# g1mv/density

Hardware: NVIDIA H100
Metric: chameleon_encode_input_GBps (higher is better)
Workload: dtype u32

## Files before the change

### density_b200/csrc/chameleon_encode.cu

```cuda
#include <cstdio>
#include "common.cuh"
#include "encode_internal.cuh"

namespace dns {
namespace cham {

constexpr int TILE_Q = 4096;
__device__ __forceinline__ bool bit_test(const uint32_t* bm, uint32_t i) { return (bm[i >> 5] >> (i & 31)) & 1u; }

constexpr int F6_THREADS = 512, F6_QPT = 8;
constexpr int F6_NW = F6_THREADS / 32, F6_WQ = 32 * F6_QPT;
static_assert(F6_THREADS * F6_QPT == TILE_Q, "tile geometry");
constexpr int F6_MB_SLOTS = 4096, F6_MB_CAP = 4;
constexpr int F6_SEC_SLOTS = 64, F6_SEC_CAP = 16;
#ifdef DNS_PHASE_TIMING
__device__ long long g_f6_ph[8];
#define F6_PH(k) { if (threadIdx.x == 0 && blockIdx.x == 77) { long long tn = clock64(); g_f6_ph[k] += tn - f6_tprev; f6_tprev = tn; } }
#define F6_PH_DECL long long f6_tprev = clock64();
#else
#define F6_PH(k)
#define F6_PH_DECL
#endif
constexpr uint32_t F6_TOUCHED = 1u << 12, F6_DROPPED = 1u << 13;
struct Flag6Smem {
// ... 247 lines not shown
                }
                if (hit) atomicOr(&S.sigw[buf][pos >> 5], 1u << (pos & 31));
            }
            f6_append_unres(unres, run_q0 + pos, r.x, &S.unres_count, unres_run);
        }
    }
    __syncthreads();
    F6_PH(3)
}

__global__ void __launch_bounds__(F6_THREADS, 1)
cham_flag_pass6(const uint32_t* __restrict__ in, uint64_t nquads, uint32_t tiles_total, uint32_t nruns,
                uint32_t* __restrict__ sigw_g, uint2* __restrict__ unres, uint32_t* __restrict__ unres_count,
                uint32_t* __restrict__ final_tab, const uint8_t* __restrict__ copymap, const Status* __restrict__ gate)
{
    if (gate && !(gate->nonquiet && !gate->converged)) return;
    extern __shared__ __align__(16) unsigned char smem_raw[];
    Flag6Smem& S = *reinterpret_cast<Flag6Smem*>(smem_raw);
    const uint32_t tid = threadIdx.x, lane = tid & 31, warp = tid >> 5;
    const uint32_t run = blockIdx.x;
    const uint64_t t_begin = (uint64_t)run * tiles_total / nruns;
    const uint64_t t_end = (uint64_t)(run + 1) * tiles_total / nruns;
    uint2* __restrict__ unres_run = unres + (size_t)run * 65536;
    const uint32_t pos0 = warp * F6_WQ + lane;
    const uint32_t ntile_run = (uint32_t)(t_end - t_begin);
    const uint64_t q_begin = t_begin * TILE_Q;
    const uint64_t q_end64 = (t_end * TILE_Q < nquads) ? t_end * TILE_Q : nquads;
    const uint32_t run_quads = q_begin < q_end64 ? (uint32_t)(q_end64 - q_begin) : 0u;
    const uint32_t* __restrict__ rin = in + q_begin;
    uint32_t* __restrict__ rsig = sigw_g + t_begin * (TILE_Q / 32);
// ... 56 lines not shown
    for (uint32_t i = tid; i < 65536; i += F6_THREADS) {
        const uint32_t v = S.tab[i];
        const uint32_t tch = (v != 0 || bit_test(S.vbit, i)) ? 0x10000u : 0u;
        final_tab[(size_t)run * 65536 + i] = v | tch;
    }
    if (tid == 0) unres_count[run] = S.unres_count < 65536u ? S.unres_count : 65536u;
#ifdef DNS_PHASE_TIMING
    if (tid == 0 && run == 77 && ntile_run) { const long long nt = ntile_run;
        printf("f6 run %u tiles %lld cycles/tile: A %lld B %lld C+deposit %lld D+S4 %lld  overflow tiles %lld dirty/tile %lld\n", run, nt, g_f6_ph[0] / nt, g_f6_ph[1] / nt,
               g_f6_ph[2] / nt, g_f6_ph[3] / nt, g_f6_ph[6], g_f6_ph[7] / nt);
        for (int k = 0; k < 8; ++k) g_f6_ph[k] = 0; }
#endif
}

__device__ __forceinline__ bool gate_open(const Status* g) { return !g || (g->nonquiet && !g->converged); }

__global__ void cham_carry_scan(const uint32_t* __restrict__ final_tab, const uint32_t* __restrict__ init, int init_untouched,
                                uint32_t nruns, uint32_t* __restrict__ carry, uint32_t* __restrict__ table_out,
                                const Status* __restrict__ gate = nullptr) {
    if (!gate_open(gate)) return;
    uint32_t hb = blockIdx.x * blockDim.x + threadIdx.x;
    if (hb >= 65536) return;
    uint32_t c = init ? init[hb] : ((hb == 0 && !init_untouched) ? 0x10000u : 0u);
    for (uint32_t r = 0; r < nruns; ++r) {
        if (carry) carry[(size_t)r * 65536 + hb] = c;
        uint32_t v = final_tab[(size_t)r * 65536 + hb];
        if (v & 0x10000u) c = v;
    }
    if (table_out) table_out[hb] = c;
}

__global__ void cham_resolve(const uint2* __restrict__ unres, const uint32_t* __restrict__ unres_count,
                             const uint32_t* __restrict__ carry, uint32_t tiles_total, uint32_t nruns,
                             uint32_t* __restrict__ sigw_g, const Status* __restrict__ gate = nullptr) {
    if (!gate_open(gate)) return;
    const uint32_t run = blockIdx.y;
    const uint32_t n = unres_count[run];
    const uint64_t run_q0 = ((uint64_t)run * tiles_total / nruns) * TILE_Q;
    for (uint32_t i = blockIdx.x * blockDim.x + threadIdx.x; i < n; i += gridDim.x * blockDim.x) {
        uint2 e = unres[(size_t)run * 65536 + i];
        uint32_t c = carry[(size_t)run * 65536 + (e.y & 0xFFFFu)];
        if ((c & 0x10000u) && (c & 0xFFFFu) == (e.y >> 16)) {
            uint64_t gq = run_q0 + e.x;
            atomicOr(&sigw_g[gq >> 5], 1u << (gq & 31));
        }
    }
}

struct ProtSmem {
    uint16_t tab[65536];
    uint32_t vbit[2048];
};

__global__ void __launch_bounds__(1024, 1)
cham_protected_pass(const uint32_t* __restrict__ in, uint64_t nbytes, const Status* __restrict__ status, int only_if_nonquiet,
                    uint32_t* __restrict__ sigw_g, uint8_t* __restrict__ copymap) {
    if (only_if_nonquiet && !(status->nonquiet && !status->converged)) return;
    extern __shared__ __align__(16) unsigned char smem_raw[];
    ProtSmem& S = *reinterpret_cast<ProtSmem*>(smem_raw);
    const uint32_t tid = threadIdx.x, lane = tid & 31;
    {
        uint4 z = make_uint4(0, 0, 0, 0);
        uint4* t4 = reinterpret_cast<uint4*>(S.tab);
        for (uint32_t i = tid; i < 65536 * 2 / 16; i += blockDim.x) t4[i] = z;
        for (uint32_t i = tid; i < 2048; i += blockDim.x) S.vbit[i] = (i == 0) ? 1u : 0u;
    }
    __syncthreads();
    if (tid >= 32) return;

    const uint64_t nquads = nbytes / 4;
    const uint64_t nblocks = (nbytes + 255) / 256;
// ... 80 lines not shown
        atomicAdd(counter, 1u);
        const unsigned int target = (epoch + 1) * nctas;
        while (atomicAdd(counter, 0u) < target) { __nanosleep(64); }
        __threadfence();
    }
    ++epoch;
    __syncthreads();
}

__device__ unsigned long long g_prot_dbg[16][2];

__global__ void __launch_bounds__(PI_THREADS)
prot_iterate(const uint32_t* __restrict__ sigw_g, uint64_t nbytes, uint64_t nblocks, uint32_t nseg, Status* __restrict__ st, int it,
             uint8_t* __restrict__ inc, uint8_t* __restrict__ cm_old, uint8_t* __restrict__ cm_new,
             uint32_t* __restrict__ in_state, uint32_t* __restrict__ out_state, uint16_t* __restrict__ ptab) {
    if (!gate_open(st)) return;
    __shared__ uint32_t s_state[1024], s_in[1024];
    __shared__ uint8_t s_inc[PSEG], s_cm[PSEG];
    __shared__ uint32_t s_cur, s_redo;
    const uint32_t tid = threadIdx.x;
    const uint64_t gtid = (uint64_t)blockIdx.x * PI_THREADS + tid, gsz = (uint64_t)gridDim.x * PI_THREADS;
    unsigned int epoch = 0;
    unsigned int* bar = &st->barrier[it & 7];

    if (sigw_g)
        for (uint64_t b = gtid; b < nblocks; b += gsz)
            if (!(it && cm_old[b])) inc[b] = (nbytes - b * 256 >= 256) && (__popc(sigw_g[2 * b]) + __popc(sigw_g[2 * b + 1]) <= 4);
    if (gtid == 0) { st->relax_changed[0] = 0; st->relax_changed[1] = 0; st->iter_changed = 0; st->pad2[0] = 0; }
    if (gtid < 16 && it == 0) { g_prot_dbg[gtid][0] = ~0ull; g_prot_dbg[gtid][1] = 0; }
    grid_barrier(bar, gridDim.x, epoch);
// ... 144 lines not shown
    }
    grid_barrier(bar, gridDim.x, epoch);
    const bool converged = *((volatile unsigned int*)&st->iter_changed) == 0;
    if (!converged || it == 0)
        for (uint64_t b = gtid; b < nblocks; b += gsz) cm_old[b] = __ldcg(&cm_new[b]);
    grid_barrier(bar, gridDim.x, epoch);
    if (gtid == 0 && converged) st->converged = 1;
}

__device__ __forceinline__ uint32_t block_out_bytes(uint64_t b, uint64_t nbytes, uint32_t hits, bool copied) {
    const uint64_t boff = b * 256;
    const uint32_t blen = (uint32_t)((nbytes - boff < 256) ? (nbytes - boff) : 256);
    return copied ? blen : 8 + blen - 2 * hits;
}

__global__ void cham_tile_sizes(const uint32_t* __restrict__ sigw_g, const uint8_t* __restrict__ copymap, uint64_t nbytes,
                                uint64_t nblocks, uint32_t ntiles, int use_copymap_if_nonquiet, int check_quiet, int assume_prev_inc,
                                Status* __restrict__ status, uint32_t* __restrict__ tile_bytes) {
    const uint32_t lane = threadIdx.x & 31;
    const uint32_t tile = blockIdx.x * (blockDim.x >> 5) + (threadIdx.x >> 5);
    if (tile >= ntiles) return;
    if (use_copymap_if_nonquiet && !check_quiet && !status->nonquiet) return;
    const bool use_cm = copymap && (!use_copymap_if_nonquiet || status->nonquiet);
    uint32_t sum = 0, incm[2];
#pragma unroll
    for (int k = 0; k < 2; ++k) {
        const uint64_t b = (uint64_t)tile * 64 + k * 32 + lane;
        uint32_t sz = 0; bool inc = false;
        if (b < nblocks) {
            const bool copied = use_cm && copymap[b];
            const uint32_t hits = __popc(sigw_g[2 * b]) + __popc(sigw_g[2 * b + 1]);
            sz = block_out_bytes(b, nbytes, hits, copied);
            inc = !copied && sz >= 256 && (nbytes - b * 256 >= 256);
        }
        sum += sz;
        incm[k] = __ballot_sync(0xFFFFFFFFu, inc);
    }
#pragma unroll
    for (int d = 16; d; d >>= 1) sum += __shfl_xor_sync(0xFFFFFFFFu, sum, d);
    if (lane == 0) tile_bytes[tile] = sum;
    if (check_quiet && lane == 0) {
        bool prev = assume_prev_inc != 0;
        if (tile > 0) {
            const uint64_t b = (uint64_t)tile * 64 - 1;
            const uint32_t hits = __popc(sigw_g[2 * b]) + __popc(sigw_g[2 * b + 1]);
            prev = (8 + 256 - 2 * hits) >= 256;
        }
        const uint64_t m = ((uint64_t)incm[1] << 32) | incm[0];
        const uint64_t pairs = m & ((m << 1) | (prev ? 1ull : 0ull));
        if (pairs) {
            atomicOr(&status->nonquiet, 1u);
            atomicMin(&status->first_nonquiet_block, (unsigned long long)tile * 64 + (__ffsll((long long)pairs) - 1));
        }
    }
}

constexpr int SCAN_T = 1024;
constexpr int SCAN_PER = 4;
constexpr int SCAN_G = SCAN_T * SCAN_PER;

__device__ __forceinline__ uint64_t block_exclusive_scan_u64(uint64_t v, uint64_t* s_warp, uint64_t* total) {
    const uint32_t lane = threadIdx.x & 31, warp = threadIdx.x >> 5;
    uint64_t incl = v;
#pragma unroll
    for (int d = 1; d < 32; d <<= 1) { uint64_t u = __shfl_up_sync(0xFFFFFFFFu, incl, d); if (lane >= (uint32_t)d) incl += u; }
    if (lane == 31) s_warp[warp] = incl;
    __syncthreads();
    if (warp == 0) {
        uint64_t w = (lane < (blockDim.x >> 5)) ? s_warp[lane] : 0;
        uint64_t wi = w;
#pragma unroll
        for (int d = 1; d < 32; d <<= 1) { uint64_t u = __shfl_up_sync(0xFFFFFFFFu, wi, d); if (lane >= (uint32_t)d) wi += u; }
        s_warp[lane] = wi - w;
        if (lane == 31) s_warp[32] = wi;
    }
    __syncthreads();
    if (total) *total = s_warp[32];
    return incl - v + s_warp[warp];
}

__global__ void __launch_bounds__(SCAN_T) scan_groups_local(const uint32_t* __restrict__ tile_bytes, uint32_t ntiles,
                                                           uint32_t* __restrict__ tile_local, uint64_t* __restrict__ group_total) {
    __shared__ uint64_t s_warp[33];
    const uint32_t base = blockIdx.x * SCAN_G + threadIdx.x * SCAN_PER;
    uint32_t v[SCAN_PER]; uint64_t sum = 0;
#pragma unroll
    for (int k = 0; k < SCAN_PER; ++k) { v[k] = (base + k < ntiles) ? tile_bytes[base + k] : 0u; sum += v[k]; }
    uint64_t tot;
    uint64_t ex = block_exclusive_scan_u64(sum, s_warp, &tot);
#pragma unroll
    for (int k = 0; k < SCAN_PER; ++k) { if (base + k < ntiles) tile_local[base + k] = (uint32_t)ex; ex += v[k]; }
    if (threadIdx.x == 0) group_total[blockIdx.x] = tot;
}

__global__ void __launch_bounds__(SCAN_T) scan_group_totals(const uint64_t* __restrict__ group_total, uint32_t ngroups,
                                                           uint64_t* __restrict__ group_off, Status* __restrict__ status,
                                                           uint64_t cap, uint64_t* __restrict__ d_out_size) {
    __shared__ uint64_t s_warp[33];
    __shared__ uint64_t s_carry;
    if (threadIdx.x == 0) s_carry = 0;
    __syncthreads();
    for (uint32_t base = 0; base < ngroups; base += SCAN_T) {
        uint32_t i = base + threadIdx.x;
        uint64_t v = (i < ngroups) ? group_total[i] : 0;
        uint64_t tot;
        uint64_t ex = block_exclusive_scan_u64(v, s_warp, &tot);
        if (i < ngroups) group_off[i] = s_carry + ex;
        __syncthreads();
        if (threadIdx.x == 0) s_carry += tot;
        __syncthreads();
    }
    if (threadIdx.x == 0) {
// ... 48 lines not shown
        if (FULL || (uint32_t)j < nv) {
            const bool hit = (fl >> j) & 1u;
            const uint32_t hsh = prod_hash(hash_prod(qs[j]));
            st_u16(p, hit ? hsh : (qs[j] & 0xFFFFu));
            if (!hit) st_u16(p + 2, qs[j] >> 16);
            p += hit ? 2 : 4;
        }
    }
}

template <bool AL16>
__global__ void __launch_bounds__(EM_THREADS)
cham_emit(const uint32_t* __restrict__ in, uint64_t nbytes, uint64_t nblocks, const uint32_t* __restrict__ sigw_g,
          const uint8_t* __restrict__ copymap, int use_copymap_if_nonquiet, const Status* __restrict__ status,
          const uint32_t* __restrict__ tile_local, const uint64_t* __restrict__ group_off, uint8_t* __restrict__ out) {
    if (status->error) return;
    __shared__ __align__(16) uint8_t s_stage[EM_STAGE];
    __shared__ uint32_t s_off[65];
    __shared__ uint32_t s_sig[128];
    __shared__ uint8_t s_copied[64];
    __shared__ uint32_t s_wsum[2];
    const uint32_t tid = threadIdx.x, lane = tid & 31, warp = tid >> 5;
    const uint32_t tile = blockIdx.x;
    const bool use_cm = copymap && (!use_copymap_if_nonquiet || status->nonquiet);
    const uint64_t tile_off = group_off[tile / SCAN_G] + tile_local[tile];
    const uint64_t nquads = nbytes / 4;
    const uint64_t tq0 = (uint64_t)tile * 4096;
    const bool full = tq0 + 4096 <= nquads;
    const uint32_t nvalid_tile = full ? 4096u : (uint32_t)(nquads > tq0 ? nquads - tq0 : 0);
    uint4 qv[4];
// ... 314 lines not shown
    L->unres = take((size_t)nruns_max * 65536 * sizeof(uint2));
    L->unres_count = take((size_t)nruns_max * sizeof(uint32_t));
    L->final_tab = take((size_t)nruns_max * 65536 * sizeof(uint32_t));
    L->carry = take((size_t)nruns_max * 65536 * sizeof(uint32_t));
    L->total = off;
    return off;
}

static cudaError_t set_smem_attrs_once() {
    static bool done = false;
    static cudaError_t err = cudaSuccess;
    if (!done) {
        err = cudaFuncSetAttribute(cham_flag_pass6, cudaFuncAttributeMaxDynamicSharedMemorySize, (int)sizeof(Flag6Smem));
        if (err == cudaSuccess)
            err = cudaFuncSetAttribute(cham_protected_pass, cudaFuncAttributeMaxDynamicSharedMemorySize, (int)sizeof(ProtSmem));
        done = true;
    }
    return err;
}

static cudaError_t prot_iterate_coop(int ctas, cudaStream_t stream, const uint32_t* sigw, uint64_t nbytes, uint64_t nblocks, uint32_t nseg, Status* st, int it,
                                     uint8_t* inc, uint8_t* cm_old, uint8_t* cm_new, uint32_t* in_state, uint32_t* out_state, uint16_t* ptab) {
    void* args[] = {&sigw, &nbytes, &nblocks, &nseg, &st, &it, &inc, &cm_old, &cm_new, &in_state, &out_state, &ptab};
    return cudaLaunchCooperativeKernel(reinterpret_cast<const void*>(prot_iterate), dim3((unsigned)ctas), dim3(PI_THREADS), args, 0, stream);
}

cudaError_t prot_debug_read(unsigned long long* out32) { return cudaMemcpyFromSymbol(out32, g_prot_dbg, sizeof(unsigned long long) * 32); }

size_t prot_state_bytes(uint64_t nseg_max) { return (2 * (nseg_max + 2) + 64) * sizeof(uint32_t) + prot_table_elems(nseg_max) * sizeof(uint16_t); }

uint32_t cham_pick_runs(size_t nbytes, int num_sms) {
    const uint64_t nblocks = (nbytes + 255) / 256;
    const uint64_t ntiles = (nblocks + 63) / 64;
    uint64_t r = ntiles / 16;
    if (r < 1) r = 1;
    if (r > (uint64_t)num_sms) r = num_sms;
    return (uint32_t)r;
}

// ... 8 lines not shown
        ntiles = (uint32_t)((nblocks + 63) / 64); ngroups = (ntiles + SCAN_G - 1) / SCAN_G;
        nseg = (uint32_t)((nblocks + PSEG - 1) / PSEG); ngrp = (nseg + PC_GROUP - 1) / PC_GROUP;
        st = at<Status>(ws, L.status); sigw = at<uint32_t>(ws, L.sigw);
        copymap = ws + L.copymap; copymap2 = ws + L.copymap2; incb = ws + L.incb;
        seg_state = at<uint32_t>(ws, L.seg_state);
        tile_bytes = at<uint32_t>(ws, L.tile_bytes); tile_local = at<uint32_t>(ws, L.tile_local);
        group_total = at<uint64_t>(ws, L.group_total); group_off = at<uint64_t>(ws, L.group_off);
        unres = at<uint2>(ws, L.unres); unres_count = at<uint32_t>(ws, L.unres_count);
        final_tab = at<uint32_t>(ws, L.final_tab); carry = at<uint32_t>(ws, L.carry);
        in_state = seg_state; out_state = seg_state + (nseg + 1);
        ptab = reinterpret_cast<uint16_t*>(seg_state + 2 * (nseg + 1));
        gin = reinterpret_cast<uint32_t*>(ptab); T = ptab + 2 * (ngrp + 2); GT = T + (size_t)nseg * PC_NC;
    }
};

static void launch_flag_pass(const ChamBufs& B, const uint8_t* d_in, uint32_t nruns, const uint8_t* copymap, const Status* gate, cudaStream_t stream,
                             uint64_t* launches) {
    cham_flag_pass6<<<nruns, F6_THREADS, sizeof(Flag6Smem), stream>>>(reinterpret_cast<const uint32_t*>(d_in), B.nquads, B.ntiles, nruns, B.sigw, B.unres,
                                                                      B.unres_count, B.final_tab, copymap, gate);
    ++*launches;
}
static void launch_carry_resolve(const ChamBufs& B, uint32_t nruns, const uint32_t* d_carry_in, const Status* gate, cudaStream_t stream,
                                 uint64_t* launches) {
    cham_carry_scan<<<65536 / 256, 256, 0, stream>>>(B.final_tab, d_carry_in, 0, nruns, B.carry, nullptr, gate);
    cham_resolve<<<dim3(32, nruns), 256, 0, stream>>>(B.unres, B.unres_count, B.carry, B.ntiles, nruns, B.sigw, gate);
    *launches += 2;
}
static void launch_export_fold(const ChamBufs& B, uint32_t nruns, uint32_t* d_table_out, const Status* gate, cudaStream_t stream, uint64_t* launches) {
    cham_carry_scan<<<65536 / 256, 256, 0, stream>>>(B.final_tab, nullptr, 1, nruns, nullptr, d_table_out, gate);
    ++*launches;
}
static cudaError_t sizes_scan_emit(const ChamBufs& B, const uint8_t* d_in, const uint8_t* copymap, int use_copymap_if_nonquiet, bool al16_ok,
                                   uint8_t* d_out, size_t cap, uint64_t* d_out_size, cudaStream_t stream, uint64_t* launches, cudaEvent_t* ev) {
    if (copymap) {
        cham_tile_sizes<<<(B.ntiles + 7) / 8, 256, 0, stream>>>(B.sigw, copymap, B.nbytes, B.nblocks, B.ntiles, use_copymap_if_nonquiet, 0, 0, B.st, B.tile_bytes);
        ++*launches;
    }
    cudaError_t e = scan_tiles_launch(B.tile_bytes, B.ntiles, B.tile_local, B.group_total, B.group_off, B.ngroups, B.st, (uint64_t)cap, d_out_size, stream);
    if (e != cudaSuccess) return e;
    *launches += 2;
    if (ev) cudaEventRecord(ev[2], stream);
    const uint32_t* in32 = reinterpret_cast<const uint32_t*>(d_in);
    if (al16_ok && (reinterpret_cast<uintptr_t>(d_in) & 15u) == 0)
        cham_emit<true><<<B.ntiles, EM_THREADS, 0, stream>>>(in32, B.nbytes, B.nblocks, B.sigw, copymap, use_copymap_if_nonquiet, B.st, B.tile_local, B.group_off, d_out);
    else
        cham_emit<false><<<B.ntiles, EM_THREADS, 0, stream>>>(in32, B.nbytes, B.nblocks, B.sigw, copymap, use_copymap_if_nonquiet, B.st, B.tile_local, B.group_off, d_out);
    ++*launches;
    if (ev) cudaEventRecord(ev[3], stream);
    return cudaGetLastError();
}

cudaError_t cham_encode_phase1(const uint8_t* d_in, size_t nbytes, uint8_t* ws, const ChamLayout& L, uint32_t nruns,
                               uint32_t* d_table_out, cudaStream_t stream, uint64_t* launches, cudaEvent_t* ev) {
    cudaError_t e = set_smem_attrs_once();
    if (e != cudaSuccess) return e;
    const ChamBufs B(ws, L, nbytes);
    e = cudaMemsetAsync(B.st, 0, sizeof(Status), stream);
    if (e == cudaSuccess) e = cudaMemsetAsync(&B.st->first_nonquiet_block, 0xFF, sizeof(unsigned long long), stream);
    if (e != cudaSuccess) return e;
    if (B.nblocks == 0) return cudaSuccess;
    if (ev) cudaEventRecord(ev[0], stream);
    launch_flag_pass(B, d_in, nruns, nullptr, nullptr, stream, launches);
    if (ev) cudaEventRecord(ev[1], stream);
    if (d_table_out) launch_export_fold(B, nruns, d_table_out, nullptr, stream, launches);
    return cudaGetLastError();
}

static cudaError_t cham_phase2_begin(const ChamBufs& B, uint32_t nruns, const uint32_t* d_carry_in, bool assume_prev_inc, cudaStream_t stream,
                                     uint64_t* launches) {
    launch_carry_resolve(B, nruns, d_carry_in, nullptr, stream, launches);
    cham_tile_sizes<<<(B.ntiles + 7) / 8, 256, 0, stream>>>(B.sigw, nullptr, B.nbytes, B.nblocks, B.ntiles, 0, 1, assume_prev_inc ? 1 : 0, B.st, B.tile_bytes);
    ++*launches;
    return cudaGetLastError();
}

static cudaError_t cham_phase2_rounds(const ChamBufs& B, const uint8_t* d_in, uint32_t nruns, const uint32_t* d_carry_in, int it_first, int it_last,
                                      bool reset_barriers, int num_sms, cudaStream_t stream, uint64_t* launches) {
    const int num_ctas = num_sms > 0 ? num_sms : 1;
    if (it_last - it_first >= 8) return cudaErrorInvalidValue;
    if (reset_barriers) {
        cudaError_t e = cudaMemsetAsync(B.st->barrier, 0, sizeof(B.st->barrier), stream);
        if (e != cudaSuccess) return e;
    }
    for (int it = it_first; it <= it_last; ++it) {
        if (it > 0) {
            launch_flag_pass(B, d_in, nruns, B.copymap, B.st, stream, launches);
            launch_carry_resolve(B, nruns, d_carry_in, B.st, stream, launches);
        }
        cudaError_t le = prot_iterate_coop(num_ctas, stream, B.sigw, B.nbytes, B.nblocks, B.nseg, B.st, it, B.incb, B.copymap, B.copymap2, B.in_state,
                                           B.out_state, B.ptab);
        if (le != cudaSuccess) return le;
        ++*launches;
    }
    return cudaGetLastError();
}

static cudaError_t cham_phase2_finish(const ChamBufs& B, const uint8_t* d_in, uint8_t* d_out, size_t cap, uint64_t* d_out_size, bool with_copy_map,
                                      bool inorder_fallback, cudaStream_t stream, uint64_t* launches, cudaEvent_t* ev) {
    if (with_copy_map && inorder_fallback) {
        cham_protected_pass<<<1, 1024, sizeof(ProtSmem), stream>>>(reinterpret_cast<const uint32_t*>(d_in), B.nbytes, B.st, 1, B.sigw, B.copymap);
        ++*launches;
    }
    return sizes_scan_emit(B, d_in, with_copy_map ? B.copymap : nullptr, 1, true, d_out, cap, d_out_size, stream, launches, ev);
}

static cudaError_t cham_phase2_needs_more(const ChamBufs& B, cudaStream_t stream, bool* more) {
    Status h;
    cudaError_t e = cudaMemcpyAsync(&h, B.st, sizeof h, cudaMemcpyDeviceToHost, stream);
    if (e == cudaSuccess) e = cudaStreamSynchronize(stream);
    if (e != cudaSuccess) return e;
    *more = h.nonquiet && !h.converged && !h.error;
    return cudaSuccess;
}

constexpr int PROT_ITERS = 4;

// ... 12 lines not shown
                               uint64_t* d_out_size, const Phase2Opts& o, int num_sms, cudaStream_t stream, uint64_t* launches) {
    if (nbytes == 0) return cudaMemsetAsync(d_out_size, 0, sizeof(uint64_t), stream);
    const ChamBufs B(ws, L, nbytes);
    cudaError_t e = cham_phase2_begin(B, nruns, o.d_carry_in, o.assume_prev_inc, stream, launches);
    if (e == cudaSuccess && o.iterate) e = cham_phase2_rounds(B, d_in, nruns, o.d_carry_in, 0, PROT_ITERS, false, num_sms, stream, launches);
    bool more = false;
    const int looks = o.max_batches + (o.give_up ? 1 : 0);
    for (int batch = 0; e == cudaSuccess && batch < looks; ++batch) {
        e = cham_phase2_needs_more(B, stream, &more);
        if (e != cudaSuccess || !more || batch >= o.max_batches) break;
        e = cham_phase2_rounds(B, d_in, nruns, o.d_carry_in, 8, 15, true, num_sms, stream, launches);
    }
    if (e != cudaSuccess) return e;
    if (o.give_up && more) { *o.give_up = true; return cudaSuccess; }
    e = cham_phase2_finish(B, d_in, d_out, cap, d_out_size, o.iterate, o.inorder_walk, stream, launches, o.ev);
    if (e == cudaSuccess && o.d_table_out) {
        launch_export_fold(B, nruns, o.d_table_out, nullptr, stream, launches);
        e = cudaGetLastError();
    }
    return e;
}

cudaError_t cham_encode_phase2(const uint8_t* d_in, size_t nbytes, uint8_t* ws, const ChamLayout& L, uint32_t nruns,
                               const uint32_t* d_carry_in, uint8_t* d_out, size_t cap, uint64_t* d_out_size,
                               bool allow_protected_fallback, bool assume_prev_inc, int num_sms, cudaStream_t stream, uint64_t* launches,
                               cudaEvent_t* ev) {
    Phase2Opts o;
    o.d_carry_in = d_carry_in; o.assume_prev_inc = assume_prev_inc; o.iterate = allow_protected_fallback; o.ev = ev;
    return cham_phase2(d_in, nbytes, ws, L, nruns, d_out, cap, d_out_size, o, num_sms, stream, launches);
}

cudaError_t cham_encode_phase2_blocking(const uint8_t* d_in, size_t nbytes, uint8_t* ws, const ChamLayout& L, uint32_t nruns, uint8_t* d_out,
                                        size_t cap, uint64_t* d_out_size, int max_batches, int num_sms, cudaStream_t stream, uint64_t* launches) {
    Phase2Opts o;
// ... 24 lines not shown

cudaError_t cham_status_accumulate(const uint8_t* ws, const ChamLayout& L, uint32_t* d_flag, cudaStream_t stream, uint64_t* launches) {
    cham_status_accumulate_k<<<1, 1, 0, stream>>>(reinterpret_cast<const Status*>(ws + L.status), d_flag);
    ++*launches;
    return cudaGetLastError();
}
cudaError_t prot_iterate_launch(const uint32_t* sigw_or_null, uint64_t nbytes, uint64_t nblocks, uint32_t nseg, Status* st, int it, uint8_t* inc,
                                uint8_t* cm_old, uint8_t* cm_new, uint32_t* in_state, uint32_t* out_state, int num_sms, cudaStream_t stream) {
    int ctas = num_sms > 0 ? num_sms : 1;
    if ((uint32_t)ctas > nseg) ctas = nseg ? (int)nseg : 1;
    return prot_iterate_coop(ctas, stream, sigw_or_null, nbytes, nblocks, nseg, st, it, inc, cm_old, cm_new, in_state, out_state,
                             reinterpret_cast<uint16_t*>(out_state + (nseg + 1)));
}
cudaError_t scan_tiles_launch(const uint32_t* tile_bytes, uint32_t ntiles, uint32_t* tile_local, uint64_t* group_total, uint64_t* group_off,
                              uint32_t ngroups, Status* st, uint64_t cap, uint64_t* d_out_size, cudaStream_t stream) {
    scan_groups_local<<<ngroups, SCAN_T, 0, stream>>>(tile_bytes, ntiles, tile_local, group_total);
    scan_group_totals<<<1, SCAN_T, 0, stream>>>(group_total, ngroups, group_off, st, cap, d_out_size);
    return cudaGetLastError();
}
cudaError_t cham_rank_fold(const uint32_t* d_tables, uint32_t rank, uint32_t* d_carry, cudaStream_t stream, uint64_t* launches) {
    cham_rank_fold_k<<<65536 / 256, 256, 0, stream>>>(d_tables, rank, d_carry);
    ++*launches;
    return cudaGetLastError();
}
cudaError_t cham_seam_words(const uint8_t* ws, const ChamLayout& L, size_t nbytes, const uint64_t* d_out_size, uint32_t* d_words, cudaStream_t stream, uint64_t* launches) {
    cham_seam_words_k<<<1, 1, 0, stream>>>(reinterpret_cast<const uint32_t*>(ws + L.sigw), nbytes, (nbytes + 255) / 256,
                                           reinterpret_cast<const Status*>(ws + L.status), d_out_size, d_words);
    ++*launches;
    return cudaGetLastError();
}
cudaError_t cham_seam_verdict(const uint32_t* d_all_words, uint32_t world, uint32_t rank, uint32_t* d_flags, uint64_t* d_total, uint64_t* d_offsets,
                              cudaStream_t stream, uint64_t* launches) {
    cham_seam_verdict_k<<<1, 1, 0, stream>>>(d_all_words, world, rank, d_flags, d_total, d_offsets);
// ... 88 lines not shown
cudaError_t cham_prot_start(uint8_t* ws, const ChamLayout& L, ProtShard* ps, uint64_t first_block, const uint64_t* d_lengths, uint32_t rank,
                            cudaStream_t stream, uint64_t* launches) {
    cham_prot_start_k<<<1, 32, 0, stream>>>(reinterpret_cast<Status*>(ws + L.status), ps, first_block, d_lengths, rank, 256u);
    ++*launches;
    return cudaGetLastError();
}
cudaError_t cham_put_u64(uint64_t* d, uint64_t v, cudaStream_t stream, uint64_t* launches) {
    cham_put_u64_k<<<1, 32, 0, stream>>>(d, v);
    ++*launches;
    return cudaGetLastError();
}

cudaError_t cham_prot_transfer(size_t nbytes, uint8_t* ws, const ChamLayout& L, uint32_t nruns, const uint32_t* d_carry_in, const ProtShard* ps,
                               int it, uint32_t* d_transfer_out, cudaStream_t stream, uint64_t* launches) {
    const ChamBufs B(ws, L, nbytes);
    if (B.nblocks) launch_carry_resolve(B, nruns, d_carry_in, B.st, stream, launches);
    return prot_transfer(cham_prot_segs(B), B.sigw, ps, it, d_transfer_out, stream, launches);
}

cudaError_t cham_prot_settle(size_t nbytes, uint8_t* ws, const ChamLayout& L, ProtShard* ps, int it, const uint32_t* d_all_transfers, uint32_t rank,
                             uint32_t* d_words, cudaStream_t stream, uint64_t* launches) {
    const ChamBufs B(ws, L, nbytes);
    return prot_settle(cham_prot_segs(B), ps, it, 0, d_all_transfers, rank, d_words, stream, launches);
}

cudaError_t cham_prot_next(const uint8_t* d_in, size_t nbytes, uint8_t* ws, const ChamLayout& L, uint32_t nruns, ProtShard* ps, int it,
                           const uint32_t* d_all_words, uint32_t world, uint32_t* d_table_out, cudaStream_t stream, uint64_t* launches) {
    const ChamBufs B(ws, L, nbytes);
    cudaError_t e = prot_commit(cham_prot_segs(B), ps, it, d_all_words, world, PROT_ROUND_WORDS, stream, launches);
    if (e != cudaSuccess) return e;
    if (d_table_out) {
        if (B.nblocks) {
            e = set_smem_attrs_once();
            if (e != cudaSuccess) return e;
            launch_flag_pass(B, d_in, nruns, B.copymap, B.st, stream, launches);
            launch_export_fold(B, nruns, d_table_out, B.st, stream, launches);
        } else {
            e = cudaMemsetAsync(d_table_out, 0, 65536 * sizeof(uint32_t), stream);
            if (e != cudaSuccess) return e;
        }
    }
    return cudaGetLastError();
}

cudaError_t cham_prot_finish(const uint8_t* d_in, size_t nbytes, uint8_t* ws, const ChamLayout& L, const ProtShard* ps, uint8_t* d_out, size_t cap,
                             uint64_t* d_out_size, uint32_t* d_seam8, cudaStream_t stream, uint64_t* launches, cudaEvent_t* ev) {
    const ChamBufs B(ws, L, nbytes);
    cudaError_t e = prot_refuse_unsettled(B.st, ps, stream, launches);
    if (e == cudaSuccess && B.nblocks) e = cham_phase2_finish(B, d_in, d_out, cap, d_out_size, true, false, stream, launches, ev);
    if (e != cudaSuccess) return e;
    return prot_seam_words(B.nblocks, B.st, d_out_size, d_seam8, stream, launches);
// ... 4 lines not shown
```

### density_b200/csrc/common.cuh

```cuda
#pragma once
#include <cuda_runtime.h>
#include <stdint.h>
#include <stddef.h>

namespace dns {

constexpr uint32_t HASH_MULT = 0x9D6EF916u;
constexpr uint32_t HASH_MULT_HALF = HASH_MULT >> 1;

constexpr uint32_t inv_odd_u32(uint32_t a) {
    uint32_t x = a;
    for (int i = 0; i < 5; ++i) x *= 2u - a * x;
    return x;
}
constexpr uint32_t HASH_MULT_HALF_INV = inv_odd_u32(HASH_MULT_HALF);
static_assert(HASH_MULT_HALF * HASH_MULT_HALF_INV == 1u, "inverse");

__host__ __device__ __forceinline__ uint32_t hash_prod(uint32_t quad) { return quad * HASH_MULT; }
__host__ __device__ __forceinline__ uint32_t prod_hash(uint32_t p) { return p >> 16; }
__host__ __device__ __forceinline__ uint32_t prod_fp(uint32_t p, uint32_t quad) { return (p & 0xFFFEu) | (quad >> 31); }
__host__ __device__ __forceinline__ uint32_t quad_from_hf(uint32_t h, uint32_t f) {
    uint32_t p = (h << 16) | (f & 0xFFFEu);
    uint32_t q31 = ((p >> 1) * HASH_MULT_HALF_INV) & 0x7FFFFFFFu;
    return q31 | (f << 31);
// ... 33 lines not shown
struct Status {
    unsigned long long out_bytes;
    unsigned int nonquiet;
    unsigned int error;
    unsigned long long first_nonquiet_block;
    unsigned int converged;
    unsigned int iter_changed;
    unsigned int barrier[8];
    unsigned int relax_changed[2];
    unsigned int pad2[2];
};

__device__ __forceinline__ uint32_t lanemask_lt() { uint32_t m; asm("mov.u32 %0, %%lanemask_lt;" : "=r"(m)); return m; }
__device__ __forceinline__ uint32_t lanemask_gt() { uint32_t m; asm("mov.u32 %0, %%lanemask_gt;" : "=r"(m)); return m; }

__device__ __forceinline__ uint32_t ld_stream_u32(const uint32_t* p) {
    uint32_t v; asm volatile("ld.global.nc.L1::no_allocate.u32 %0, [%1];" : "=r"(v) : "l"(p)); return v;
}
__device__ __forceinline__ void st_u16(uint8_t* p, uint32_t v) { *reinterpret_cast<uint16_t*>(p) = (uint16_t)v; }

}
```

Before: 484.0.

## Add programmatic dependent launch chain and restructure carry/resolve and tile-size kernels

Adds griddepcontrol wait/trigger to most encode kernels and launches them with programmatic stream serialization, so each kernel's launch overlaps the tail of the previous one. The carry scan now writes 16-bit fingerprints plus a packed touched-bit array. The resolve kernel runs one CTA per run, loads that run's carry table into shared memory and looks entries up there. Tile sizing processes several tiles per warp with vectorized signature loads, and launch errors are now propagated. The cost is more complex launch code and dependence on correct PDL ordering, since early triggers could expose races.

```diff
diff --git a/density_b200/csrc/chameleon_encode.cu b/density_b200/csrc/chameleon_encode.cu
--- a/density_b200/csrc/chameleon_encode.cu
+++ b/density_b200/csrc/chameleon_encode.cu
@@ -1,4 +1,5 @@
 #include <cstdio>
+#include <utility>
 #include "common.cuh"
 #include "encode_internal.cuh"
 
@@ -285,6 +286,7 @@
                 uint32_t* __restrict__ sigw_g, uint2* __restrict__ unres, uint32_t* __restrict__ unres_count,
                 uint32_t* __restrict__ final_tab, const uint8_t* __restrict__ copymap, const Status* __restrict__ gate)
 {
+    pdl_wait();
     if (gate && !(gate->nonquiet && !gate->converged)) return;
     extern __shared__ __align__(16) unsigned char smem_raw[];
     Flag6Smem& S = *reinterpret_cast<Flag6Smem*>(smem_raw);
@@ -371,35 +373,73 @@
 }
 
 __device__ __forceinline__ bool gate_open(const Status* g) { return !g || (g->nonquiet && !g->converged); }
-
-__global__ void cham_carry_scan(const uint32_t* __restrict__ final_tab, const uint32_t* __restrict__ init, int init_untouched,
-                                uint32_t nruns, uint32_t* __restrict__ carry, uint32_t* __restrict__ table_out,
-                                const Status* __restrict__ gate = nullptr) {
+__host__ __device__ __forceinline__ uint32_t* carry_touched(uint32_t* carry, uint32_t nruns) { return carry + (size_t)nruns * (65536 / 2); }
+
+constexpr int CS_THREADS = 256;
+static_assert(65536 % CS_THREADS == 0, "every warp of the carry scan is full (ballot)");
+__global__ void __launch_bounds__(CS_THREADS)
+cham_carry_scan(const uint32_t* __restrict__ final_tab, const uint32_t* __restrict__ init, int init_untouched,
+                uint32_t nruns, uint32_t* __restrict__ carry, uint32_t* __restrict__ table_out, const Status* __restrict__ gate) {
+    pdl_wait();
+    pdl_trigger();
     if (!gate_open(gate)) return;
-    uint32_t hb = blockIdx.x * blockDim.x + threadIdx.x;
-    if (hb >= 65536) return;
+    const uint32_t hb = blockIdx.x * CS_THREADS + threadIdx.x;
+    uint16_t* __restrict__ cfp = reinterpret_cast<uint16_t*>(carry);
+    uint32_t* __restrict__ ctb = carry ? carry_touched(carry, nruns) : nullptr;
     uint32_t c = init ? init[hb] : ((hb == 0 && !init_untouched) ? 0x10000u : 0u);
     for (uint32_t r = 0; r < nruns; ++r) {
-        if (carry) carry[(size_t)r * 65536 + hb] = c;
-        uint32_t v = final_tab[(size_t)r * 65536 + hb];
+        if (carry) {
+            cfp[(size_t)r * 65536 + hb] = (uint16_t)c;
+            const uint32_t tb = __ballot_sync(0xFFFFFFFFu, (c & 0x10000u) != 0);
+            if ((threadIdx.x & 31) == 0) ctb[(size_t)r * 2048 + (hb >> 5)] = tb;
+        }
+        const uint32_t v = final_tab[(size_t)r * 65536 + hb];
         if (v & 0x10000u) c = v;
     }
     if (table_out) table_out[hb] = c;
 }
 
-__global__ void cham_resolve(const uint2* __restrict__ unres, const uint32_t* __restrict__ unres_count,
-                             const uint32_t* __restrict__ carry, uint32_t tiles_total, uint32_t nruns,
-                             uint32_t* __restrict__ sigw_g, const Status* __restrict__ gate = nullptr) {
+constexpr int RS_THREADS = 1024, RS_PER = 8;
+struct ResolveSmem {
+    uint16_t fp[65536];
+    uint32_t touched[2048];
+};
+__global__ void __launch_bounds__(RS_THREADS, 1)
+cham_resolve(const uint2* __restrict__ unres, const uint32_t* __restrict__ unres_count,
+             const uint32_t* __restrict__ carry, uint32_t tiles_total, uint32_t nruns,
+             uint32_t* __restrict__ sigw_g, const Status* __restrict__ gate) {
+    pdl_wait();
+    pdl_trigger();
     if (!gate_open(gate)) return;
-    const uint32_t run = blockIdx.y;
+    extern __shared__ __align__(16) unsigned char smem_raw[];
+    ResolveSmem& S = *reinterpret_cast<ResolveSmem*>(smem_raw);
+    const uint32_t run = blockIdx.x, tid = threadIdx.x;
+    {
+        const uint4* __restrict__ sfp = reinterpret_cast<const uint4*>(carry) + (size_t)run * (65536 * 2 / 16);
+        const uint4* __restrict__ stb = reinterpret_cast<const uint4*>(carry_touched(const_cast<uint32_t*>(carry), nruns)) + (size_t)run * (2048 * 4 / 16);
+        uint4* dfp = reinterpret_cast<uint4*>(S.fp);
+        uint4 v[65536 * 2 / 16 / RS_THREADS];
+#pragma unroll
+        for (int k = 0; k < 65536 * 2 / 16 / RS_THREADS; ++k) v[k] = sfp[k * RS_THREADS + tid];
+#pragma unroll
+        for (int k = 0; k < 65536 * 2 / 16 / RS_THREADS; ++k) dfp[k * RS_THREADS + tid] = v[k];
+        if (tid < 2048 * 4 / 16) reinterpret_cast<uint4*>(S.touched)[tid] = stb[tid];
+    }
+    __syncthreads();
     const uint32_t n = unres_count[run];
     const uint64_t run_q0 = ((uint64_t)run * tiles_total / nruns) * TILE_Q;
-    for (uint32_t i = blockIdx.x * blockDim.x + threadIdx.x; i < n; i += gridDim.x * blockDim.x) {
-        uint2 e = unres[(size_t)run * 65536 + i];
-        uint32_t c = carry[(size_t)run * 65536 + (e.y & 0xFFFFu)];
-        if ((c & 0x10000u) && (c & 0xFFFFu) == (e.y >> 16)) {
-            uint64_t gq = run_q0 + e.x;
-            atomicOr(&sigw_g[gq >> 5], 1u << (gq & 31));
+    const uint2* __restrict__ ul = unres + (size_t)run * 65536;
+    for (uint32_t i0 = tid; i0 < n; i0 += RS_THREADS * RS_PER) {
+        uint2 e[RS_PER];
+#pragma unroll
+        for (int k = 0; k < RS_PER; ++k) e[k] = (i0 + k * RS_THREADS < n) ? ul[i0 + k * RS_THREADS] : make_uint2(0, 0);
+#pragma unroll
+        for (int k = 0; k < RS_PER; ++k) {
+            const uint32_t h = e[k].y & 0xFFFFu;
+            if (i0 + k * RS_THREADS < n && bit_test(S.touched, h) && S.fp[h] == (e[k].y >> 16)) {
+                const uint64_t gq = run_q0 + e[k].x;
+                atomicOr(&sigw_g[gq >> 5], 1u << (gq & 31));
+            }
         }
     }
 }
@@ -412,6 +452,8 @@
 __global__ void __launch_bounds__(1024, 1)
 cham_protected_pass(const uint32_t* __restrict__ in, uint64_t nbytes, const Status* __restrict__ status, int only_if_nonquiet,
                     uint32_t* __restrict__ sigw_g, uint8_t* __restrict__ copymap) {
+    pdl_wait();
+    pdl_trigger();
     if (only_if_nonquiet && !(status->nonquiet && !status->converged)) return;
     extern __shared__ __align__(16) unsigned char smem_raw[];
     ProtSmem& S = *reinterpret_cast<ProtSmem*>(smem_raw);
@@ -522,6 +564,7 @@
 prot_iterate(const uint32_t* __restrict__ sigw_g, uint64_t nbytes, uint64_t nblocks, uint32_t nseg, Status* __restrict__ st, int it,
              uint8_t* __restrict__ inc, uint8_t* __restrict__ cm_old, uint8_t* __restrict__ cm_new,
              uint32_t* __restrict__ in_state, uint32_t* __restrict__ out_state, uint16_t* __restrict__ ptab) {
+    pdl_wait();
     if (!gate_open(st)) return;
     __shared__ uint32_t s_state[1024], s_in[1024];
     __shared__ uint8_t s_inc[PSEG], s_cm[PSEG];
@@ -696,43 +739,61 @@
     return copied ? blen : 8 + blen - 2 * hits;
 }
 
-__global__ void cham_tile_sizes(const uint32_t* __restrict__ sigw_g, const uint8_t* __restrict__ copymap, uint64_t nbytes,
-                                uint64_t nblocks, uint32_t ntiles, int use_copymap_if_nonquiet, int check_quiet, int assume_prev_inc,
-                                Status* __restrict__ status, uint32_t* __restrict__ tile_bytes) {
+constexpr int TS_THREADS = 256, TS_TILES = 4;
+constexpr int TS_TILES_PER_CTA = TS_THREADS / 32 * TS_TILES;
+__global__ void __launch_bounds__(TS_THREADS)
+cham_tile_sizes(const uint32_t* __restrict__ sigw_g, const uint8_t* __restrict__ copymap, uint64_t nbytes,
+                uint64_t nblocks, uint32_t ntiles, int use_copymap_if_nonquiet, int check_quiet, int assume_prev_inc,
+                Status* __restrict__ status, uint32_t* __restrict__ tile_bytes) {
+    pdl_wait();
+    pdl_trigger();
+    if (use_copymap_if_nonquiet && !check_quiet && !status->nonquiet) return;
     const uint32_t lane = threadIdx.x & 31;
-    const uint32_t tile = blockIdx.x * (blockDim.x >> 5) + (threadIdx.x >> 5);
-    if (tile >= ntiles) return;
-    if (use_copymap_if_nonquiet && !check_quiet && !status->nonquiet) return;
+    const uint32_t tile0 = (blockIdx.x * (TS_THREADS / 32) + (threadIdx.x >> 5)) * TS_TILES;
     const bool use_cm = copymap && (!use_copymap_if_nonquiet || status->nonquiet);
-    uint32_t sum = 0, incm[2];
-#pragma unroll
-    for (int k = 0; k < 2; ++k) {
-        const uint64_t b = (uint64_t)tile * 64 + k * 32 + lane;
-        uint32_t sz = 0; bool inc = false;
-        if (b < nblocks) {
-            const bool copied = use_cm && copymap[b];
-            const uint32_t hits = __popc(sigw_g[2 * b]) + __popc(sigw_g[2 * b + 1]);
-            sz = block_out_bytes(b, nbytes, hits, copied);
-            inc = !copied && sz >= 256 && (nbytes - b * 256 >= 256);
-        }
-        sum += sz;
-        incm[k] = __ballot_sync(0xFFFFFFFFu, inc);
-    }
-#pragma unroll
-    for (int d = 16; d; d >>= 1) sum += __shfl_xor_sync(0xFFFFFFFFu, sum, d);
-    if (lane == 0) tile_bytes[tile] = sum;
-    if (check_quiet && lane == 0) {
-        bool prev = assume_prev_inc != 0;
-        if (tile > 0) {
-            const uint64_t b = (uint64_t)tile * 64 - 1;
-            const uint32_t hits = __popc(sigw_g[2 * b]) + __popc(sigw_g[2 * b + 1]);
-            prev = (8 + 256 - 2 * hits) >= 256;
-        }
-        const uint64_t m = ((uint64_t)incm[1] << 32) | incm[0];
-        const uint64_t pairs = m & ((m << 1) | (prev ? 1ull : 0ull));
-        if (pairs) {
-            atomicOr(&status->nonquiet, 1u);
-            atomicMin(&status->first_nonquiet_block, (unsigned long long)tile * 64 + (__ffsll((long long)pairs) - 1));
+    const uint2* __restrict__ sig2 = reinterpret_cast<const uint2*>(sigw_g);
+    uint2 sg[TS_TILES][2];
+#pragma unroll
+    for (int t = 0; t < TS_TILES; ++t)
+#pragma unroll
+        for (int k = 0; k < 2; ++k) {
+            const uint64_t b = (uint64_t)(tile0 + t) * 64 + k * 32 + lane;
+            sg[t][k] = (tile0 + t < ntiles && b < nblocks) ? sig2[b] : make_uint2(0, 0);
+        }
+#pragma unroll
+    for (int t = 0; t < TS_TILES; ++t) {
+        const uint32_t tile = tile0 + t;
+        if (tile >= ntiles) break;
+        uint32_t sum = 0, incm[2];
+#pragma unroll
+        for (int k = 0; k < 2; ++k) {
+            const uint64_t b = (uint64_t)tile * 64 + k * 32 + lane;
+            uint32_t sz = 0; bool inc = false;
+            if (b < nblocks) {
+                const bool copied = use_cm && copymap[b];
+                const uint32_t hits = __popc(sg[t][k].x) + __popc(sg[t][k].y);
+                sz = block_out_bytes(b, nbytes, hits, copied);
+                inc = !copied && sz >= 256 && (nbytes - b * 256 >= 256);
+            }
+            sum += sz;
+            incm[k] = __ballot_sync(0xFFFFFFFFu, inc);
+        }
+#pragma unroll
+        for (int d = 16; d; d >>= 1) sum += __shfl_xor_sync(0xFFFFFFFFu, sum, d);
+        if (lane == 0) tile_bytes[tile] = sum;
+        if (check_quiet && lane == 0) {
+            bool prev = assume_prev_inc != 0;
+            if (tile > 0) {
+                const uint64_t b = (uint64_t)tile * 64 - 1;
+                const uint32_t hits = __popc(sigw_g[2 * b]) + __popc(sigw_g[2 * b + 1]);
+                prev = (8 + 256 - 2 * hits) >= 256;
+            }
+            const uint64_t m = ((uint64_t)incm[1] << 32) | incm[0];
+            const uint64_t pairs = m & ((m << 1) | (prev ? 1ull : 0ull));
+            if (pairs) {
+                atomicOr(&status->nonquiet, 1u);
+                atomicMin(&status->first_nonquiet_block, (unsigned long long)tile * 64 + (__ffsll((long long)pairs) - 1));
+            }
         }
     }
 }
@@ -763,6 +824,8 @@
 
 __global__ void __launch_bounds__(SCAN_T) scan_groups_local(const uint32_t* __restrict__ tile_bytes, uint32_t ntiles,
                                                            uint32_t* __restrict__ tile_local, uint64_t* __restrict__ group_total) {
+    pdl_wait();
+    pdl_trigger();
     __shared__ uint64_t s_warp[33];
     const uint32_t base = blockIdx.x * SCAN_G + threadIdx.x * SCAN_PER;
     uint32_t v[SCAN_PER]; uint64_t sum = 0;
@@ -778,6 +841,8 @@
 __global__ void __launch_bounds__(SCAN_T) scan_group_totals(const uint64_t* __restrict__ group_total, uint32_t ngroups,
                                                            uint64_t* __restrict__ group_off, Status* __restrict__ status,
                                                            uint64_t cap, uint64_t* __restrict__ d_out_size) {
+    pdl_wait();
+    pdl_trigger();
     __shared__ uint64_t s_warp[33];
     __shared__ uint64_t s_carry;
     if (threadIdx.x == 0) s_carry = 0;
@@ -856,6 +921,7 @@
 cham_emit(const uint32_t* __restrict__ in, uint64_t nbytes, uint64_t nblocks, const uint32_t* __restrict__ sigw_g,
           const uint8_t* __restrict__ copymap, int use_copymap_if_nonquiet, const Status* __restrict__ status,
           const uint32_t* __restrict__ tile_local, const uint64_t* __restrict__ group_off, uint8_t* __restrict__ out) {
+    pdl_wait();
     if (status->error) return;
     __shared__ __align__(16) uint8_t s_stage[EM_STAGE];
     __shared__ uint32_t s_off[65];
@@ -1200,15 +1266,31 @@
         err = cudaFuncSetAttribute(cham_flag_pass6, cudaFuncAttributeMaxDynamicSharedMemorySize, (int)sizeof(Flag6Smem));
         if (err == cudaSuccess)
             err = cudaFuncSetAttribute(cham_protected_pass, cudaFuncAttributeMaxDynamicSharedMemorySize, (int)sizeof(ProtSmem));
+        if (err == cudaSuccess)
+            err = cudaFuncSetAttribute(cham_resolve, cudaFuncAttributeMaxDynamicSharedMemorySize, (int)sizeof(ResolveSmem));
         done = true;
     }
     return err;
+}
+
+template <typename... KArgs, typename... Args>
+static cudaError_t launch_pdl(void (*kernel)(KArgs...), dim3 grid, dim3 block, size_t smem, cudaStream_t stream, bool cooperative,
+                              Args&&... args) {
+    cudaLaunchAttribute at[2];
+    at[0].id = cudaLaunchAttributeProgrammaticStreamSerialization;
+    at[0].val.programmaticStreamSerializationAllowed = 1;
+    at[1].id = cudaLaunchAttributeCooperative;
+    at[1].val.cooperative = 1;
+    cudaLaunchConfig_t cfg = {};
+    cfg.gridDim = grid; cfg.blockDim = block; cfg.dynamicSmemBytes = smem; cfg.stream = stream;
+    cfg.attrs = at; cfg.numAttrs = cooperative ? 2 : 1;
+    return cudaLaunchKernelEx(&cfg, kernel, std::forward<Args>(args)...);
 }
 
 static cudaError_t prot_iterate_coop(int ctas, cudaStream_t stream, const uint32_t* sigw, uint64_t nbytes, uint64_t nblocks, uint32_t nseg, Status* st, int it,
                                      uint8_t* inc, uint8_t* cm_old, uint8_t* cm_new, uint32_t* in_state, uint32_t* out_state, uint16_t* ptab) {
-    void* args[] = {&sigw, &nbytes, &nblocks, &nseg, &st, &it, &inc, &cm_old, &cm_new, &in_state, &out_state, &ptab};
-    return cudaLaunchCooperativeKernel(reinterpret_cast<const void*>(prot_iterate), dim3((unsigned)ctas), dim3(PI_THREADS), args, 0, stream);
+    return launch_pdl(prot_iterate, dim3((unsigned)ctas), dim3(PI_THREADS), 0, stream, true, sigw, nbytes, nblocks, nseg, st, it, inc, cm_old,
+                      cm_new, in_state, out_state, ptab);
 }
 
 cudaError_t prot_debug_read(unsigned long long* out32) { return cudaMemcpyFromSymbol(out32, g_prot_dbg, sizeof(unsigned long long) * 32); }
@@ -1247,40 +1329,59 @@
     }
 };
 
-static void launch_flag_pass(const ChamBufs& B, const uint8_t* d_in, uint32_t nruns, const uint8_t* copymap, const Status* gate, cudaStream_t stream,
-                             uint64_t* launches) {
-    cham_flag_pass6<<<nruns, F6_THREADS, sizeof(Flag6Smem), stream>>>(reinterpret_cast<const uint32_t*>(d_in), B.nquads, B.ntiles, nruns, B.sigw, B.unres,
-                                                                      B.unres_count, B.final_tab, copymap, gate);
-    ++*launches;
-}
-static void launch_carry_resolve(const ChamBufs& B, uint32_t nruns, const uint32_t* d_carry_in, const Status* gate, cudaStream_t stream,
-                                 uint64_t* launches) {
-    cham_carry_scan<<<65536 / 256, 256, 0, stream>>>(B.final_tab, d_carry_in, 0, nruns, B.carry, nullptr, gate);
-    cham_resolve<<<dim3(32, nruns), 256, 0, stream>>>(B.unres, B.unres_count, B.carry, B.ntiles, nruns, B.sigw, gate);
+static cudaError_t launch_flag_pass(const ChamBufs& B, const uint8_t* d_in, uint32_t nruns, const uint8_t* copymap, const Status* gate,
+                                    cudaStream_t stream, uint64_t* launches) {
+    const uint32_t* in32 = reinterpret_cast<const uint32_t*>(d_in);
+    cudaError_t e = cudaSuccess;
+    if (gate)
+        e = launch_pdl(cham_flag_pass6, dim3(nruns), dim3(F6_THREADS), sizeof(Flag6Smem), stream, false, in32, B.nquads, B.ntiles, nruns, B.sigw,
+                       B.unres, B.unres_count, B.final_tab, copymap, gate);
+    else
+        cham_flag_pass6<<<nruns, F6_THREADS, sizeof(Flag6Smem), stream>>>(in32, B.nquads, B.ntiles, nruns, B.sigw, B.unres, B.unres_count, B.final_tab,
+                                                                          copymap, gate);
+    ++*launches;
+    return e;
+}
+static cudaError_t launch_carry_resolve(const ChamBufs& B, uint32_t nruns, const uint32_t* d_carry_in, const Status* gate, cudaStream_t stream,
+                                        uint64_t* launches) {
+    cudaError_t e = set_smem_attrs_once();
+    if (e == cudaSuccess)
+        e = launch_pdl(cham_carry_scan, dim3(65536 / CS_THREADS), dim3(CS_THREADS), 0, stream, false, B.final_tab, d_carry_in, 0, nruns, B.carry,
+                       (uint32_t*)nullptr, gate);
+    if (e == cudaSuccess)
+        e = launch_pdl(cham_resolve, dim3(nruns), dim3(RS_THREADS), sizeof(ResolveSmem), stream, false, B.unres, B.unres_count, B.carry, B.ntiles, nruns,
+                       B.sigw, gate);
     *launches += 2;
-}
-static void launch_export_fold(const ChamBufs& B, uint32_t nruns, uint32_t* d_table_out, const Status* gate, cudaStream_t stream, uint64_t* launches) {
-    cham_carry_scan<<<65536 / 256, 256, 0, stream>>>(B.final_tab, nullptr, 1, nruns, nullptr, d_table_out, gate);
-    ++*launches;
+    return e;
+}
+static cudaError_t launch_export_fold(const ChamBufs& B, uint32_t nruns, uint32_t* d_table_out, const Status* gate, cudaStream_t stream,
+                                      uint64_t* launches) {
+    ++*launches;
+    return launch_pdl(cham_carry_scan, dim3(65536 / CS_THREADS), dim3(CS_THREADS), 0, stream, false, B.final_tab, (const uint32_t*)nullptr, 1, nruns,
+                      (uint32_t*)nullptr, d_table_out, gate);
+}
+static cudaError_t launch_tile_sizes(const ChamBufs& B, const uint8_t* copymap, int use_copymap_if_nonquiet, int check_quiet, int assume_prev_inc,
+                                     cudaStream_t stream, uint64_t* launches) {
+    ++*launches;
+    return launch_pdl(cham_tile_sizes, dim3((B.ntiles + TS_TILES_PER_CTA - 1) / TS_TILES_PER_CTA), dim3(TS_THREADS), 0, stream, false, B.sigw,
+                      copymap, B.nbytes, B.nblocks, B.ntiles, use_copymap_if_nonquiet, check_quiet, assume_prev_inc, B.st, B.tile_bytes);
 }
 static cudaError_t sizes_scan_emit(const ChamBufs& B, const uint8_t* d_in, const uint8_t* copymap, int use_copymap_if_nonquiet, bool al16_ok,
                                    uint8_t* d_out, size_t cap, uint64_t* d_out_size, cudaStream_t stream, uint64_t* launches, cudaEvent_t* ev) {
-    if (copymap) {
-        cham_tile_sizes<<<(B.ntiles + 7) / 8, 256, 0, stream>>>(B.sigw, copymap, B.nbytes, B.nblocks, B.ntiles, use_copymap_if_nonquiet, 0, 0, B.st, B.tile_bytes);
-        ++*launches;
-    }
-    cudaError_t e = scan_tiles_launch(B.tile_bytes, B.ntiles, B.tile_local, B.group_total, B.group_off, B.ngroups, B.st, (uint64_t)cap, d_out_size, stream);
+    cudaError_t e = cudaSuccess;
+    if (copymap) e = launch_tile_sizes(B, copymap, use_copymap_if_nonquiet, 0, 0, stream, launches);
+    if (e == cudaSuccess)
+        e = scan_tiles_launch(B.tile_bytes, B.ntiles, B.tile_local, B.group_total, B.group_off, B.ngroups, B.st, (uint64_t)cap, d_out_size, stream);
     if (e != cudaSuccess) return e;
     *launches += 2;
     if (ev) cudaEventRecord(ev[2], stream);
     const uint32_t* in32 = reinterpret_cast<const uint32_t*>(d_in);
-    if (al16_ok && (reinterpret_cast<uintptr_t>(d_in) & 15u) == 0)
-        cham_emit<true><<<B.ntiles, EM_THREADS, 0, stream>>>(in32, B.nbytes, B.nblocks, B.sigw, copymap, use_copymap_if_nonquiet, B.st, B.tile_local, B.group_off, d_out);
-    else
-        cham_emit<false><<<B.ntiles, EM_THREADS, 0, stream>>>(in32, B.nbytes, B.nblocks, B.sigw, copymap, use_copymap_if_nonquiet, B.st, B.tile_local, B.group_off, d_out);
+    const bool al16 = al16_ok && (reinterpret_cast<uintptr_t>(d_in) & 15u) == 0;
+    e = launch_pdl(al16 ? cham_emit<true> : cham_emit<false>, dim3(B.ntiles), dim3(EM_THREADS), 0, stream, false, in32, B.nbytes, B.nblocks, B.sigw,
+                   copymap, use_copymap_if_nonquiet, B.st, B.tile_local, B.group_off, d_out);
     ++*launches;
     if (ev) cudaEventRecord(ev[3], stream);
-    return cudaGetLastError();
+    return e != cudaSuccess ? e : cudaGetLastError();
 }
 
 cudaError_t cham_encode_phase1(const uint8_t* d_in, size_t nbytes, uint8_t* ws, const ChamLayout& L, uint32_t nruns,
@@ -1293,18 +1394,17 @@
     if (e != cudaSuccess) return e;
     if (B.nblocks == 0) return cudaSuccess;
     if (ev) cudaEventRecord(ev[0], stream);
-    launch_flag_pass(B, d_in, nruns, nullptr, nullptr, stream, launches);
+    e = launch_flag_pass(B, d_in, nruns, nullptr, nullptr, stream, launches);
     if (ev) cudaEventRecord(ev[1], stream);
-    if (d_table_out) launch_export_fold(B, nruns, d_table_out, nullptr, stream, launches);
-    return cudaGetLastError();
+    if (e == cudaSuccess && d_table_out) e = launch_export_fold(B, nruns, d_table_out, nullptr, stream, launches);
+    return e != cudaSuccess ? e : cudaGetLastError();
 }
 
 static cudaError_t cham_phase2_begin(const ChamBufs& B, uint32_t nruns, const uint32_t* d_carry_in, bool assume_prev_inc, cudaStream_t stream,
                                      uint64_t* launches) {
-    launch_carry_resolve(B, nruns, d_carry_in, nullptr, stream, launches);
-    cham_tile_sizes<<<(B.ntiles + 7) / 8, 256, 0, stream>>>(B.sigw, nullptr, B.nbytes, B.nblocks, B.ntiles, 0, 1, assume_prev_inc ? 1 : 0, B.st, B.tile_bytes);
-    ++*launches;
-    return cudaGetLastError();
+    cudaError_t e = launch_carry_resolve(B, nruns, d_carry_in, nullptr, stream, launches);
+    if (e == cudaSuccess) e = launch_tile_sizes(B, nullptr, 0, 1, assume_prev_inc ? 1 : 0, stream, launches);
+    return e != cudaSuccess ? e : cudaGetLastError();
 }
 
 static cudaError_t cham_phase2_rounds(const ChamBufs& B, const uint8_t* d_in, uint32_t nruns, const uint32_t* d_carry_in, int it_first, int it_last,
@@ -1317,8 +1417,9 @@
     }
     for (int it = it_first; it <= it_last; ++it) {
         if (it > 0) {
-            launch_flag_pass(B, d_in, nruns, B.copymap, B.st, stream, launches);
-            launch_carry_resolve(B, nruns, d_carry_in, B.st, stream, launches);
+            cudaError_t e = launch_flag_pass(B, d_in, nruns, B.copymap, B.st, stream, launches);
+            if (e == cudaSuccess) e = launch_carry_resolve(B, nruns, d_carry_in, B.st, stream, launches);
+            if (e != cudaSuccess) return e;
         }
         cudaError_t le = prot_iterate_coop(num_ctas, stream, B.sigw, B.nbytes, B.nblocks, B.nseg, B.st, it, B.incb, B.copymap, B.copymap2, B.in_state,
                                            B.out_state, B.ptab);
@@ -1331,8 +1432,10 @@
 static cudaError_t cham_phase2_finish(const ChamBufs& B, const uint8_t* d_in, uint8_t* d_out, size_t cap, uint64_t* d_out_size, bool with_copy_map,
                                       bool inorder_fallback, cudaStream_t stream, uint64_t* launches, cudaEvent_t* ev) {
     if (with_copy_map && inorder_fallback) {
-        cham_protected_pass<<<1, 1024, sizeof(ProtSmem), stream>>>(reinterpret_cast<const uint32_t*>(d_in), B.nbytes, B.st, 1, B.sigw, B.copymap);
+        cudaError_t e = launch_pdl(cham_protected_pass, dim3(1), dim3(1024), sizeof(ProtSmem), stream, false, reinterpret_cast<const uint32_t*>(d_in),
+                                   (uint64_t)B.nbytes, (const Status*)B.st, 1, B.sigw, B.copymap);
         ++*launches;
+        if (e != cudaSuccess) return e;
     }
     return sizes_scan_emit(B, d_in, with_copy_map ? B.copymap : nullptr, 1, true, d_out, cap, d_out_size, stream, launches, ev);
 }
@@ -1375,10 +1478,7 @@
     if (e != cudaSuccess) return e;
     if (o.give_up && more) { *o.give_up = true; return cudaSuccess; }
     e = cham_phase2_finish(B, d_in, d_out, cap, d_out_size, o.iterate, o.inorder_walk, stream, launches, o.ev);
-    if (e == cudaSuccess && o.d_table_out) {
-        launch_export_fold(B, nruns, o.d_table_out, nullptr, stream, launches);
-        e = cudaGetLastError();
-    }
+    if (e == cudaSuccess && o.d_table_out) e = launch_export_fold(B, nruns, o.d_table_out, nullptr, stream, launches);
     return e;
 }
 
@@ -1433,9 +1533,9 @@
 }
 cudaError_t scan_tiles_launch(const uint32_t* tile_bytes, uint32_t ntiles, uint32_t* tile_local, uint64_t* group_total, uint64_t* group_off,
                               uint32_t ngroups, Status* st, uint64_t cap, uint64_t* d_out_size, cudaStream_t stream) {
-    scan_groups_local<<<ngroups, SCAN_T, 0, stream>>>(tile_bytes, ntiles, tile_local, group_total);
-    scan_group_totals<<<1, SCAN_T, 0, stream>>>(group_total, ngroups, group_off, st, cap, d_out_size);
-    return cudaGetLastError();
+    cudaError_t e = launch_pdl(scan_groups_local, dim3(ngroups), dim3(SCAN_T), 0, stream, false, tile_bytes, ntiles, tile_local, group_total);
+    if (e == cudaSuccess) e = launch_pdl(scan_group_totals, dim3(1), dim3(SCAN_T), 0, stream, false, group_total, ngroups, group_off, st, cap, d_out_size);
+    return e;
 }
 cudaError_t cham_rank_fold(const uint32_t* d_tables, uint32_t rank, uint32_t* d_carry, cudaStream_t stream, uint64_t* launches) {
     cham_rank_fold_k<<<65536 / 256, 256, 0, stream>>>(d_tables, rank, d_carry);
@@ -1554,7 +1654,10 @@
 cudaError_t cham_prot_transfer(size_t nbytes, uint8_t* ws, const ChamLayout& L, uint32_t nruns, const uint32_t* d_carry_in, const ProtShard* ps,
                                int it, uint32_t* d_transfer_out, cudaStream_t stream, uint64_t* launches) {
     const ChamBufs B(ws, L, nbytes);
-    if (B.nblocks) launch_carry_resolve(B, nruns, d_carry_in, B.st, stream, launches);
+    if (B.nblocks) {
+        const cudaError_t e = launch_carry_resolve(B, nruns, d_carry_in, B.st, stream, launches);
+        if (e != cudaSuccess) return e;
+    }
     return prot_transfer(cham_prot_segs(B), B.sigw, ps, it, d_transfer_out, stream, launches);
 }
 
@@ -1573,8 +1676,9 @@
         if (B.nblocks) {
             e = set_smem_attrs_once();
             if (e != cudaSuccess) return e;
-            launch_flag_pass(B, d_in, nruns, B.copymap, B.st, stream, launches);
-            launch_export_fold(B, nruns, d_table_out, B.st, stream, launches);
+            e = launch_flag_pass(B, d_in, nruns, B.copymap, B.st, stream, launches);
+            if (e == cudaSuccess) e = launch_export_fold(B, nruns, d_table_out, B.st, stream, launches);
+            if (e != cudaSuccess) return e;
         } else {
             e = cudaMemsetAsync(d_table_out, 0, 65536 * sizeof(uint32_t), stream);
             if (e != cudaSuccess) return e;
diff --git a/density_b200/csrc/common.cuh b/density_b200/csrc/common.cuh
--- a/density_b200/csrc/common.cuh
+++ b/density_b200/csrc/common.cuh
@@ -71,6 +71,9 @@
 __device__ __forceinline__ uint32_t lanemask_lt() { uint32_t m; asm("mov.u32 %0, %%lanemask_lt;" : "=r"(m)); return m; }
 __device__ __forceinline__ uint32_t lanemask_gt() { uint32_t m; asm("mov.u32 %0, %%lanemask_gt;" : "=r"(m)); return m; }
 
+__device__ __forceinline__ void pdl_wait() { asm volatile("griddepcontrol.wait;" ::: "memory"); }
+__device__ __forceinline__ void pdl_trigger() { asm volatile("griddepcontrol.launch_dependents;" ::: "memory"); }
+
 __device__ __forceinline__ uint32_t ld_stream_u32(const uint32_t* p) {
     uint32_t v; asm volatile("ld.global.nc.L1::no_allocate.u32 %0, [%1];" : "=r"(v) : "l"(p)); return v;
 }
```

New measurement: 495.6 (median of 6 runs). 2.4% higher.
